# popgenmethods/smcpp

Hardware: AMD Instinct MI355X
Metric: E-step loglik-evals/sec (100 Mbp, M=64, n=20) (higher is better)
Workload: dtype f64 state + f32 scans (mixed)

## Files before the change

smcpp_amd/csrc/chains_ss.hpp:

```cpp
#pragma once

namespace smcpp_dev {

struct SsArgs {
    int M, Mp, nchunks, pass, K, nlds;
    const Chunk *chunks;
    const Chunk *chunks_b;
    int nchunks_b;
    const int *tasks;
    const int2 *rowdesc;
    const double *E;
    const float *pi_f;
    const double *f_dc, *f_g, *f_cg, *f_b, *f_a, *f_d;
    const double *b_dc, *b_g, *b_b, *b_a;
    double c0;
    float *alpha;
    double *beta, *cnorm;
    float *ends_f, *used_f;
    double *ends_b, *used_b;
    int *changed_f, *changed_b;
    int *endchg_f, *endchg_b;
    float eps_f;
    double eps_b;
    int full_f, full_b;
// ... 531 lines not shown
}
#define SS_NBE_ " row_mask:0xf bank_mask:0xf\n"
__device__ __forceinline__ float ss_jump_16(float acc, float X, const float *r) {
    asm volatile("s_nop 1\n"
                 "v_fmac_f32_dpp %0, %1, %2 row_newbcast:0" SS_NBE_ "v_fmac_f32_dpp %0, %1, %3 row_newbcast:1" SS_NBE_
                 "v_fmac_f32_dpp %0, %1, %4 row_newbcast:2" SS_NBE_ "v_fmac_f32_dpp %0, %1, %5 row_newbcast:3" SS_NBE_
                 "v_fmac_f32_dpp %0, %1, %6 row_newbcast:4" SS_NBE_ "v_fmac_f32_dpp %0, %1, %7 row_newbcast:5" SS_NBE_
                 "v_fmac_f32_dpp %0, %1, %8 row_newbcast:6" SS_NBE_ "v_fmac_f32_dpp %0, %1, %9 row_newbcast:7" SS_NBE_
                 "v_fmac_f32_dpp %0, %1, %10 row_newbcast:8" SS_NBE_ "v_fmac_f32_dpp %0, %1, %11 row_newbcast:9" SS_NBE_
                 "v_fmac_f32_dpp %0, %1, %12 row_newbcast:10" SS_NBE_ "v_fmac_f32_dpp %0, %1, %13 row_newbcast:11" SS_NBE_
                 "v_fmac_f32_dpp %0, %1, %14 row_newbcast:12" SS_NBE_ "v_fmac_f32_dpp %0, %1, %15 row_newbcast:13" SS_NBE_
                 "v_fmac_f32_dpp %0, %1, %16 row_newbcast:14" SS_NBE_ "v_fmac_f32_dpp %0, %1, %17 row_newbcast:15" SS_NBE_
                 : "+v"(acc)
                 : "v"(X), "v"(r[0]), "v"(r[1]), "v"(r[2]), "v"(r[3]), "v"(r[4]), "v"(r[5]), "v"(r[6]), "v"(r[7]), "v"(r[8]), "v"(r[9]),
                   "v"(r[10]), "v"(r[11]), "v"(r[12]), "v"(r[13]), "v"(r[14]), "v"(r[15]));
    return acc;
}
#undef SS_NBE_
__device__ __forceinline__ float ss_jump_mv(const SsJumpR &j, float x) {
    const unsigned xi = __builtin_bit_cast(unsigned, x);
    const auto s16 = __builtin_amdgcn_permlane16_swap(xi, xi, false, false);
    const auto sa = __builtin_amdgcn_permlane32_swap(s16[0], s16[0], false, false);
    const auto sb = __builtin_amdgcn_permlane32_swap(s16[1], s16[1], false, false);
    const float a0 = ss_jump_16(0.f, __builtin_bit_cast(float, (unsigned)sa[0]), j.r);
    const float a1 = ss_jump_16(0.f, __builtin_bit_cast(float, (unsigned)sb[0]), j.r + 16);
    const float a2 = ss_jump_16(0.f, __builtin_bit_cast(float, (unsigned)sa[1]), j.r + 32);
    const float a3 = ss_jump_16(0.f, __builtin_bit_cast(float, (unsigned)sb[1]), j.r + 48);
    return (a0 + a1) + (a2 + a3);
}
__device__ __forceinline__ int ss_jump_run(const SsJumpR &j, float &x, int t, int span) {
    const float df = (float)j.d;
    const int nj = (span - t) >> j.sh;
    for (int q = 0; q < nj; ++q) x = __builtin_fmaf(df, x, ss_jump_mv(j, x));
    return t + (nj << (j.sh & 15));
}

__global__ __launch_bounds__(256) void k_ss_jump_tables(SsArgs a, int slot, float *__restrict__ tf, float *__restrict__ tt, double *__restrict__ diag) {
    const int lane = threadIdx.x & 63, i = blockIdx.x * 4 + (threadIdx.x >> 6);
    SsFwdC<1> cst;
    ss_load_fwd<1>(a, lane, cst);
    double e[1], x[1], y[1], S;
    e[0] = a.E[(size_t)slot * 64 + lane];
    x[0] = (lane == i && i < a.M) ? 1.0 : 0.0;
    for (int t = 0; t < a.jump; ++t) {
        ss_fwd_step<1>(cst, x, e, y, S);
        x[0] = y[0];
    }
    const float v = lane == i ? 0.f : (float)x[0];
    tf[lane * 64 + i] = v;
    tt[i * 64 + (63 - lane)] = v;
    if (lane == i) diag[i] = x[0];
}

template <int NPL, bool ALLLDS, bool JMP = false>
__device__ __forceinline__ void ss_fwd_light_rows(const SsArgs &a, const double *sE, long long base, int first, int last, int lane, float (&x)[NPL]);
template <int NPL, bool ALLLDS, bool JMP = false>
__device__ __forceinline__ void ss_bwd_light_rows(const SsArgs &a, const double *sE, long long base, int rhi, int rlo, int lane, float (&b)[NPL]);

template <int NPL, bool RERUN, bool HYB, bool ALLLDS, bool MIX = false, bool H32 = false>
__device__ __forceinline__ void ss_forward_wave(const SsArgs &a, const double *sE, int c, int lane) {
    constexpr int MS = 64 * NPL;
    const int M = a.M, Mp = a.Mp, pass = a.pass;
    const Chunk ch = ss_uniform_chunk(a.chunks[c]);
    float *end_cur = a.ends_f + ((size_t)(pass & 1) * a.nchunks + c) * Mp;
    const float *end_prev = a.ends_f + ((size_t)((pass + 1) & 1) * a.nchunks + c) * Mp;
    int st[NPL];
    bool live[NPL], stor[NPL];
#pragma unroll
    for (int k = 0; k < NPL; ++k) { st[k] = lane * NPL + k; live[k] = st[k] < M; stor[k] = st[k] < Mp; }
    if (RERUN && ch.first && !a.full_f) {
#pragma unroll
        for (int k = 0; k < NPL; ++k) if (stor[k]) end_cur[st[k]] = end_prev[st[k]];
        return;
    }
    double x[NPL];
    {
        const float *src = (ch.first || !RERUN) ? a.pi_f : a.ends_f + ((size_t)((pass + 1) & 1) * a.nchunks + (c - 1)) * Mp;
#pragma unroll
        for (int k = 0; k < NPL; ++k) x[k] = live[k] ? (double)src[st[k]] : 0.0;
    }
    const bool halo = !RERUN && !HYB && a.halo && ch.h0 < ch.r0;
    const int rbeg = halo ? ch.h1 : ch.r0;
    const int jst = ch.r0 - rbeg;
    if (halo && ch.h0 < ch.h1) {
        float xf[NPL];
#pragma unroll
        for (int k = 0; k < NPL; ++k) xf[k] = (float)x[k];
        if (NPL == 1 && !HYB && a.jump) ss_fwd_light_rows<NPL, ALLLDS, NPL == 1 && !HYB>(a, sE, ch.base, ch.h0, ch.h1, lane, xf);
        else ss_fwd_light_rows<NPL, ALLLDS>(a, sE, ch.base, ch.h0, ch.h1, lane, xf);
#pragma unroll
        for (int k = 0; k < NPL; ++k) x[k] = live[k] ? (double)xf[k] : 0.0;
        if (jst == 0) {
            double part = 0.0;
#pragma unroll
            for (int k = 0; k < NPL; ++k) part += x[k];
            const double iv = 1.0 / wave_sum_dpp(part);
#pragma unroll
            for (int k = 0; k < NPL; ++k) {
                const float an = live[k] ? fmaxf((float)(x[k] * iv), ss_floor_at<NPL>(a, ch.base + ch.r0 + 1)) : 0.f;
                x[k] = (double)an;
                if (stor[k]) a.used_f[(size_t)c * Mp + st[k]] = an;
            }
        }
    }
    if (RERUN && !a.full_f) {
        bool diff = false;
#pragma unroll
        for (int k = 0; k < NPL; ++k)
            if (live[k]) {
                const float u = a.used_f[(size_t)c * Mp + st[k]];
                if (!(fabsf((float)x[k] - u) <= a.eps_f * fabsf(u))) diff = true;
            }
        if (!__any(diff)) {
#pragma unroll
            for (int k = 0; k < NPL; ++k) if (stor[k]) end_cur[st[k]] = end_prev[st[k]];
            return;
        }
    }
    if (!halo) {
#pragma unroll
        for (int k = 0; k < NPL; ++k) if (stor[k]) a.used_f[(size_t)c * Mp + st[k]] = (float)x[k];
    }
    if (lane == 0) a.changed_f[pass] = 1;
    if (ch.first) {
#pragma unroll
        for (int k = 0; k < NPL; ++k) if (stor[k]) a.alpha[(size_t)ch.base * Mp + st[k]] = (float)x[k];
        if (lane == 0) a.cnorm[ch.base] = 1.0;
    }
    SsFwdC<NPL> cst;
    ss_load_fwd<NPL>(a, lane, cst);
    SsDescStream rd = ss_desc_stream(a.rowdesc + ch.base + rbeg + 1);
    const int nrows = ch.r1 - rbeg;
    ss_desc_t d1, d2;
    ss_desc_first<1>(rd, d1, d2);
    float *arow = a.alpha + (size_t)(ch.base + rbeg) * Mp;
    double *crow = a.cnorm + ch.base + rbeg;
    float *ap[NPL];
#pragma unroll
    for (int k = 0; k < NPL; ++k) ap[k] = arow + st[k];
    int cacc = 0;
    auto cflush = [&](int jhi) {
        const int jj = (jhi & ~63) + lane;
        if (jj <= jhi && jj > jst && jj > 0) crow[jj] = (double)__builtin_bit_cast(float, cacc);
    };
    double e[NPL];
    ss_emission<NPL, false, ALLLDS>(a, sE, d1.x & 0xFFFF, lane, e);
    constexpr bool hyb = HYB && NPL == 1;
    const double *tab = sE + (size_t)a.nlds * MS;
    SsEigC ec;
    SsHotRows<16> hot;
    int hot_ek = -1;
    if (hyb) {
        ss_load_eig(a, lane, ec);
        if (Mp == 32) { hot_ek = a.hot_ek; ss_eig_rows<16>(ec, tab, Mp, hot_ek, 0, hot.a, hot.b); }
    }
    double *sxw = const_cast<double *>(tab) + (size_t)a.nk_lds * (a.dirsplit ? 2 : 4) * Mp * (Mp + 1) + (threadIdx.x >> 6) * 64;
    bool merged = false;
    const long long t0c = __builtin_readcyclecounter(), t0r = __builtin_amdgcn_s_memrealtime();
    long long npos = 0;
    ss_vm_drain();
    for (int j = 0; j < nrows; ++j) {
        const int jl = j & 63;
        const ss_desc_t d0 = d1;
        d1 = d2; d2 = ss_desc_fetch<1>(rd, d1.x);
        const int span = d0.y;
        const int ekr = (d0.x >> 16) & 0xFF;
        const float flo = NPL >= 2 ? ss_floor_of<NPL>(d0.x) : 1e-10f;
        npos += span;
        if (MIX && jl == 0 && j > 0) cflush(j - 1);
        const int slot_n = d1.x & 0xFFFF;
        double en[NPL];
        ss_emission<NPL, false, ALLLDS>(a, sE, slot_n, lane, en);
        if (hyb && span > a.hyb_th) {
            const double S = wave_sum_dpp(x[0]);
            const double inv = rcp_f64(S);
            double xin = x[0] * inv;
            if (j > 0) {
                const float an = live[0] ? fmaxf((float)xin, flo) : 0.f;
                if (RERUN && !a.full_f && (j & 15) == 0 && j >= 16) {
                    bool bad = false;
                    if (live[0]) {
                        const float old = arow[(size_t)j * Mp + st[0]];
                        if (!(fabsf(an - old) <= a.eps_f * fabsf(old))) bad = true;
                    }
                    if (!__any(bad)) { merged = true; break; }
                }
                if (stor[0]) arow[(size_t)j * Mp + st[0]] = an;
                if (lane == 0) crow[j] = S;
                xin = (double)an;
            }
            const double xo = ss_eig_apply(a, ec, tab, Mp, ekr, 0, sxw, lane, xin, span, hot, hot_ek);
            x[0] = live[0] ? xo : 0.0;
#pragma unroll
            for (int k = 0; k < NPL; ++k) e[k] = en[k];
            continue;
        }
        double y[NPL], S;
        ss_fwd_step<NPL, MIX, MIX && H32>(cst, x, e, y, S);
        double inv;
        if (MIX) {
            const double r0 = (double)__builtin_amdgcn_rcpf((float)S);
            inv = __builtin_fma(__builtin_fma(-S, r0, 1.0), r0, r0);
        } else inv = rcp_f64(S);
        double fb[NPL];
#pragma unroll
        for (int k = 0; k < NPL; ++k) fb[k] = 0.0;
        if (j > 0) {
            float an[NPL];
#pragma unroll
            for (int k = 0; k < NPL; ++k) {
                const double xs = x[k] * inv;
                an[k] = live[k] ? fmaxf((float)xs, flo) : 0.f;
                fb[k] = (double)an[k] - xs;
            }
            if (RERUN && !a.full_f && (j & 15) == 0 && j >= 16) {
                bool bad = false;
#pragma unroll
                for (int k = 0; k < NPL; ++k)
                    if (live[k]) {
                        const float old = MIX ? *ap[k] : arow[(size_t)j * Mp + st[k]];
                        if (!(fabsf(an[k] - old) <= a.eps_f * fabsf(old))) bad = true;
                    }
                if (!__any(bad)) { merged = true; if (MIX) cflush(j - 1); break; }
            }
            if (j > jst) {
                if (MIX) {
#pragma unroll
                    for (int k = 0; k < NPL; ++k) if (stor[k]) *ap[k] = an[k];
                    cacc = lane == jl ? __builtin_bit_cast(int, (float)S) : cacc;
                } else {
#pragma unroll
                    for (int k = 0; k < NPL; ++k) if (stor[k]) arow[(size_t)j * Mp + st[k]] = an[k];
                    if (lane == 0) crow[j] = S;
                }
            } else if (j == jst) {
#pragma unroll
                for (int k = 0; k < NPL; ++k) if (stor[k]) a.used_f[(size_t)c * Mp + st[k]] = an[k];
            }
        }
#pragma unroll
        for (int k = 0; k < NPL; ++k) {
            double ed = e[k] * cst.d[k];
            if (span == 1) { const double edf = (double)(float)ed; y[k] = __builtin_fma(edf - ed, x[k], y[k]); ed = edf; }
            x[k] = __builtin_fma(ed, fb[k], y[k] * inv);
        }
        {
            double S2;
            int t = 1;
            for (; t + 1 < span; t += 2) {
                ss_fwd_step<NPL, MIX, MIX && H32>(cst, x, e, y, S2);
#pragma unroll
                for (int k = 0; k < NPL; ++k) x[k] = y[k];
                ss_fwd_step<NPL, MIX, MIX && H32>(cst, x, e, y, S2);
#pragma unroll
                for (int k = 0; k < NPL; ++k) x[k] = y[k];
            }
            if (t < span) {
                ss_fwd_step<NPL, MIX, MIX && H32>(cst, x, e, y, S2);
#pragma unroll
                for (int k = 0; k < NPL; ++k) x[k] = y[k];
            }
        }
#pragma unroll
        for (int k = 0; k < NPL; ++k) e[k] = en[k];
        if (MIX) {
#pragma unroll
            for (int k = 0; k < NPL; ++k) ap[k] += Mp;
        }
    }
    if (MIX && !merged && nrows > 0) cflush(nrows - 1);
    if (a.dbg && !RERUN && c == 1 && lane == 0) {
        a.dbg[0] = __builtin_readcyclecounter() - t0c; a.dbg[1] = __builtin_amdgcn_s_memrealtime() - t0r;
        a.dbg[2] = npos; a.dbg[3] = nrows;
    }
    if (merged) {
#pragma unroll
        for (int k = 0; k < NPL; ++k) if (stor[k]) end_cur[st[k]] = end_prev[st[k]];
        return;
    }
    {
        double part = 0.0;
#pragma unroll
        for (int k = 0; k < NPL; ++k) part += x[k];
        const double S = wave_sum_dpp(part);
        const double inv = 1.0 / S;
#pragma unroll
        for (int k = 0; k < NPL; ++k) {
            const float an = live[k] ? fmaxf((float)(x[k] * inv), ss_floor_at<NPL>(a, ch.base + ch.r1 + 1)) : 0.f;
            if (stor[k]) { a.alpha[(size_t)(ch.base + ch.r1) * Mp + st[k]] = an; end_cur[st[k]] = an; }
        }
        if (lane == 0) { a.cnorm[ch.base + ch.r1] = S; a.endchg_f[pass] = 1; }
    }
}

template <int NPL, bool RERUN, bool HYB, bool ALLLDS, bool MIX = false, bool H32 = false>
__device__ __forceinline__ void ss_backward_wave(const SsArgs &a, const double *sE, int c, int lane) {
    constexpr int MS = 64 * NPL;
    const int M = a.M, Mp = a.Mp, pass = a.pass;
    const Chunk ch = ss_uniform_chunk(a.chunks_b[c]);
    double *end_cur = a.ends_b + ((size_t)(pass & 1) * a.nchunks_b + c) * Mp;
    const double *end_prev = a.ends_b + ((size_t)((pass + 1) & 1) * a.nchunks_b + c) * Mp;
    int st[NPL];
    bool live[NPL], stor[NPL];
#pragma unroll
    for (int k = 0; k < NPL; ++k) { st[k] = MS - 1 - (lane * NPL + k); live[k] = st[k] < M; stor[k] = st[k] < Mp; }
    if (RERUN && ch.last && !a.full_b) {
#pragma unroll
        for (int k = 0; k < NPL; ++k) if (stor[k]) end_cur[st[k]] = end_prev[st[k]];
        return;
    }
    double b[NPL];
    {
        const bool fresh = ch.last || !RERUN;
        const double *src = a.ends_b + ((size_t)((pass + 1) & 1) * a.nchunks_b + (fresh ? c : c + 1)) * Mp;
#pragma unroll
        for (int k = 0; k < NPL; ++k) b[k] = live[k] ? (fresh ? 1.0 / (double)M : src[st[k]]) : 0.0;
    }
    const bool halo = !RERUN && !HYB && a.halo && ch.h0 > ch.r1;
    const int rend = halo ? ch.h1 : ch.r1;
    const int jst = rend - ch.r1;
    if (halo && ch.h0 > ch.h1) {
        float bf_[NPL];
#pragma unroll
        for (int k = 0; k < NPL; ++k) bf_[k] = (float)b[k];
        if (NPL == 1 && !HYB && a.jump) ss_bwd_light_rows<NPL, ALLLDS, NPL == 1 && !HYB>(a, sE, ch.base, ch.h0, ch.h1, lane, bf_);
        else ss_bwd_light_rows<NPL, ALLLDS>(a, sE, ch.base, ch.h0, ch.h1, lane, bf_);
        float pt = 0.f;
#pragma unroll
        for (int k = 0; k < NPL; ++k) pt += live[k] ? bf_[k] : 0.f;
        const float iv = 1.f / wave_sum_dpp(pt);
#pragma unroll
        for (int k = 0; k < NPL; ++k) b[k] = live[k] ? (double)(bf_[k] * iv) : 0.0;
    }
    if (RERUN && !a.full_b) {
        bool diff = false;
#pragma unroll
        for (int k = 0; k < NPL; ++k)
            if (live[k]) {
                const double u = a.used_b[(size_t)c * Mp + st[k]];
                if (!(fabs(b[k] - u) <= a.eps_b * fabs(u))) diff = true;
            }
        if (!__any(diff)) {
#pragma unroll
            for (int k = 0; k < NPL; ++k) if (stor[k]) end_cur[st[k]] = end_prev[st[k]];
            return;
        }
    }
    if (!halo) {
#pragma unroll
        for (int k = 0; k < NPL; ++k) if (stor[k]) a.used_b[(size_t)c * Mp + st[k]] = b[k];
    }
    if (lane == 0) a.changed_b[pass] = 1;
    SsBwdC<NPL> cst;
    ss_load_bwd<NPL>(a, lane, cst);
    SsDescStream rd = ss_desc_stream(a.rowdesc + ch.base + rend);
    const int nrows = rend - ch.r0;
    ss_desc_t d1, d2;
    ss_desc_first<-1>(rd, d1, d2);
    double *brow = a.beta + (size_t)(ch.base + rend) * Mp;
    double *bp[NPL];
#pragma unroll
    for (int k = 0; k < NPL; ++k) bp[k] = brow + st[k];
    double e[NPL];
    ss_emission<NPL, true, ALLLDS>(a, sE, d1.x & 0xFFFF, lane, e);
    constexpr bool hyb = HYB && NPL == 1;
    const double *tab = sE + (size_t)a.nlds * MS;
    SsEigC ec;
    SsHotRows<16> hot;
    int hot_ek = -1;
    if (hyb) {
        ss_load_eig(a, 63 - lane, ec);
        if (Mp == 32) { hot_ek = a.hot_ek; ss_eig_rows<16>(ec, tab, Mp, hot_ek, 2, hot.a, hot.b); }
    }
    double *sxw = const_cast<double *>(tab) + (size_t)a.nk_lds * (a.dirsplit ? 2 : 4) * Mp * (Mp + 1) + (threadIdx.x >> 6) * 64;
    bool merged = false;
    const long long t0c = __builtin_readcyclecounter(), t0r = __builtin_amdgcn_s_memrealtime();
    long long npos = 0;
    ss_vm_drain();
    for (int j = 0; j < nrows; ++j) {
        const ss_desc_t d0 = d1;
        d1 = d2; d2 = ss_desc_fetch<-1>(rd, d1.x);
        const int span = d0.y;
        const int ekr = (d0.x >> 16) & 0xFF;
        npos += span;
        const int slot_n = d1.x & 0xFFFF;
        double en[NPL];
        ss_emission<NPL, true, ALLLDS>(a, sE, slot_n, lane, en);
        if (RERUN && !a.full_b && (j & 15) == 0 && j >= 16) {
            bool bad = false;
#pragma unroll
            for (int k = 0; k < NPL; ++k)
                if (live[k]) {
                    const double old = MIX ? *bp[k] : brow[-(ptrdiff_t)j * Mp + st[k]];
                    if (!(fabs(b[k] - old) <= a.eps_b * fabs(old))) bad = true;
                }
            if (!__any(bad)) { merged = true; break; }
        }
        if (halo && j == jst) {
            double part = 0.0;
#pragma unroll
            for (int k = 0; k < NPL; ++k) part += live[k] ? b[k] : 0.0;
            const double iv = 1.0 / wave_sum_dpp(part);
#pragma unroll
            for (int k = 0; k < NPL; ++k) {
                b[k] = live[k] ? b[k] * iv : 0.0;
                if (stor[k]) a.used_b[(size_t)c * Mp + st[k]] = b[k];
            }
        }
        if (j >= jst) {
#pragma unroll
            for (int k = 0; k < NPL; ++k) if (stor[k]) { if (MIX) *bp[k] = b[k]; else brow[-(ptrdiff_t)j * Mp + st[k]] = b[k]; }
        }
        if (hyb && span > a.hyb_th) {
            const double bin = live[0] ? b[0] : 0.0;
            double bo = ss_eig_apply(a, ec, tab, Mp, ekr, 2, sxw, 63 - lane, bin, span, hot, hot_ek);
            bo = live[0] ? bo : 0.0;
            b[0] = bo * rcp_f64(wave_sum_dpp(bo));
#pragma unroll
            for (int k = 0; k < NPL; ++k) e[k] = en[k];
            continue;
        }
        double y[NPL];
        float Sw;
        ss_bwd_step<NPL, MIX, MIX && H32>(cst, b, e, y, Sw);
        const double inv = (double)__builtin_amdgcn_rcpf(Sw);
#pragma unroll
        for (int k = 0; k < NPL; ++k) b[k] = y[k] * inv;
        {
            float S2;
            int t = 1;
            for (; t + 1 < span; t += 2) {
                ss_bwd_step<NPL, MIX, MIX && H32>(cst, b, e, y, S2);
#pragma unroll
                for (int k = 0; k < NPL; ++k) b[k] = y[k];
                ss_bwd_step<NPL, MIX, MIX && H32>(cst, b, e, y, S2);
#pragma unroll
                for (int k = 0; k < NPL; ++k) b[k] = y[k];
            }
            if (t < span) {
                ss_bwd_step<NPL, MIX, MIX && H32>(cst, b, e, y, S2);
#pragma unroll
                for (int k = 0; k < NPL; ++k) b[k] = y[k];
            }
        }
#pragma unroll
        for (int k = 0; k < NPL; ++k) e[k] = en[k];
        if (MIX) {
#pragma unroll
            for (int k = 0; k < NPL; ++k) bp[k] -= Mp;
        }
    }
    if (a.dbg && !RERUN && c == 1 && lane == 0) {
        a.dbg[4] = __builtin_readcyclecounter() - t0c; a.dbg[5] = __builtin_amdgcn_s_memrealtime() - t0r;
        a.dbg[6] = npos; a.dbg[7] = nrows;
    }
    if (merged) {
#pragma unroll
        for (int k = 0; k < NPL; ++k) if (stor[k]) end_cur[st[k]] = end_prev[st[k]];
        return;
    }
    {
        double part = 0.0;
#pragma unroll
        for (int k = 0; k < NPL; ++k) part += live[k] ? b[k] : 0.0;
        const double S = wave_sum_dpp(part);
#pragma unroll
        for (int k = 0; k < NPL; ++k) {
            const double bf = live[k] ? b[k] / S : 0.0;
            if (stor[k]) { end_cur[st[k]] = bf; if (ch.first) a.beta[(size_t)ch.base * Mp + st[k]] = bf; }
        }
        if (lane == 0) a.endchg_b[pass] = 1;
    }
}

template <int NPL>
struct SsLightC { float dc[NPL], g[NPL], cg[NPL], b[NPL], a[NPL], cumA[NPL], lv[6], c15, c31, c0; };

template <int NPL, bool BWD>
__device__ __forceinline__ void ss_load_light(const SsArgs &a, int lane, SsLightC<NPL> &c) {
    double cum = 1.0;
#pragma unroll
    for (int k = 0; k < NPL; ++k) {
        const int p = lane * NPL + k;
        c.dc[k] = (float)(BWD ? a.b_dc[p] : a.f_dc[p]);
        c.g[k] = (float)(BWD ? a.b_g[p] : a.f_g[p]);
        c.cg[k] = BWD ? 0.f : (float)a.f_cg[p];
        c.b[k] = (float)(BWD ? a.b_b[p] : a.f_b[p]);
        const double av = BWD ? a.b_a[p] : a.f_a[p];
        c.a[k] = (float)av;
        cum *= av;
        c.cumA[k] = (float)cum;
    }
    double lv[6];
    ss_levels(cum, lane, lv);
#pragma unroll
    for (int q = 0; q < 6; ++q) c.lv[q] = (float)lv[q];
    const int row = lane >> 4;
// ... 68 lines not shown
    const float LIp = dpp0<DPP_WSHR1>(z_);
    if (NPL == 1) {
        out[0] = e[0] * __builtin_fmaf(c.dc[0], x[0], __builtin_fmaf(c.g[0], S, __builtin_fmaf(c.cg[0], p_, LIp)));
        return;
    }
    const float lex = p_ - lp[NPL - 1];
#pragma unroll
    for (int k = 0; k < NPL; ++k) {
        const float incl = lex + lp[k];
        const float Z = (k == 0) ? LIp : __builtin_fmaf(c.cumA[k - 1 < 0 ? 0 : k - 1], LIp, w[k - 1 < 0 ? 0 : k - 1]);
        out[k] = e[k] * __builtin_fmaf(c.dc[k], x[k], __builtin_fmaf(c.g[k], S, __builtin_fmaf(c.cg[k], incl, Z)));
    }
}

template <int NPL, bool H32 = false>
__device__ __forceinline__ void ss_bwd_step_f(const SsLightC<NPL> &c, const float (&bv)[NPL], const float (&e)[NPL],
                                              float (&out)[NPL], float &Sw) {
    float w[NPL], lg[NPL], u[NPL], lf[NPL];
#pragma unroll
    for (int k = 0; k < NPL; ++k) w[k] = e[k] * bv[k];
    lg[0] = c.g[0] * w[0];
    u[0] = w[0];
    lf[0] = w[0];
#pragma unroll
    for (int k = 1; k < NPL; ++k) {
        lg[k] = __builtin_fmaf(c.g[k], w[k], lg[k - 1]);
        u[k] = __builtin_fmaf(c.a[k], u[k - 1], w[k]);
        lf[k] = lf[k - 1] + w[k];
    }
    float p_ = lg[NPL - 1], z_ = u[NPL - 1], f_ = lf[NPL - 1];
    ss_light_scan3<H32>(p_, z_, f_, c.lv, c.c15, c.c31);
    const float Gtot = lane_get(p_, 63);
    Sw = lane_get(f_, 63);
    const float LIp = dpp0<DPP_WSHR1>(z_);
    if (NPL == 1) {
        out[0] = __builtin_fmaf(c.dc[0], w[0], (Gtot - p_) + __builtin_fmaf(c.c0, f_, c.b[0] * LIp));
        return;
    }
    const float lexg = p_ - lg[NPL - 1], lexf = f_ - lf[NPL - 1];
#pragma unroll
    for (int k = 0; k < NPL; ++k) {
        const float inclG = lexg + lg[k], inclW = lexf + lf[k];
        const float V = (k == 0) ? LIp : __builtin_fmaf(c.cumA[k - 1 < 0 ? 0 : k - 1], LIp, u[k - 1 < 0 ? 0 : k - 1]);
        out[k] = __builtin_fmaf(c.dc[k], w[k], (Gtot - inclG) + __builtin_fmaf(c.c0, inclW, c.b[k] * V));
    }
}

template <int NPL, bool BWD, bool ALLLDS>
__device__ __forceinline__ void ss_emission_f(const SsArgs &a, const double *sE, int slot, int lane, float (&e)[NPL]) {
    double ed[NPL];
    ss_emission<NPL, BWD, ALLLDS>(a, sE, slot, lane, ed);
#pragma unroll
    for (int k = 0; k < NPL; ++k) e[k] = (float)ed[k];
}

template <int NPL, bool ALLLDS, bool JMP>
__device__ __forceinline__ void ss_fwd_light_rows(const SsArgs &a, const double *sE, long long base, int first, int last, int lane,
                                                  float (&x)[NPL]) {
    SsLightC<NPL> cst;
    ss_load_light<NPL, false>(a, lane, cst);
    SsDescStream rd = ss_desc_stream(a.rowdesc + base + first + 1);
    const int nrows = last - first;
    ss_desc_t d1, d2;
    ss_desc_first<1>(rd, d1, d2);
    float e[NPL];
    ss_emission_f<NPL, false, ALLLDS>(a, sE, d1.x & 0xFFFF, lane, e);
    SsJumpR jr;
    jr.P = 0; jr.sh = 31;
    if constexpr (JMP) ss_jump_load<false>(a, lane, jr);
    ss_vm_drain();
    for (int j = 0; j < nrows; ++j) {
        const ss_desc_t d0 = d1;
        d1 = d2; d2 = ss_desc_fetch<1>(rd, d1.x);
        const int span = d0.y;
        const bool jrow = JMP && (d0.x & SS_ROW_JUMP);
        const int slot_n = d1.x & 0xFFFF;
        float en[NPL], y[NPL], S;
        ss_emission_f<NPL, false, ALLLDS>(a, sE, slot_n, lane, en);
        ss_fwd_step_f<NPL>(cst, x, e, y, S);
        const float inv = __builtin_amdgcn_rcpf(S);
#pragma unroll
        for (int k = 0; k < NPL; ++k) x[k] = y[k] * inv;
        float S2;
        int t = 1;
        if constexpr (JMP) { if (__builtin_expect(jrow, 0)) t = ss_jump_run(jr, x[0], t, span); }
        for (; t + 1 < span; t += 2) {
            ss_fwd_step_f<NPL>(cst, x, e, y, S2);
#pragma unroll
            for (int k = 0; k < NPL; ++k) x[k] = y[k];
            ss_fwd_step_f<NPL>(cst, x, e, y, S2);
#pragma unroll
            for (int k = 0; k < NPL; ++k) x[k] = y[k];
        }
        if (t < span) {
            ss_fwd_step_f<NPL>(cst, x, e, y, S2);
#pragma unroll
            for (int k = 0; k < NPL; ++k) x[k] = y[k];
        }
#pragma unroll
        for (int k = 0; k < NPL; ++k) e[k] = en[k];
    }
}
template <int NPL, bool ALLLDS, bool JMP>
__device__ __forceinline__ void ss_bwd_light_rows(const SsArgs &a, const double *sE, long long base, int rhi, int rlo, int lane,
                                                  float (&b)[NPL]) {
    SsLightC<NPL> cst;
    ss_load_light<NPL, true>(a, lane, cst);
    SsDescStream rd = ss_desc_stream(a.rowdesc + base + rhi);
    const int nrows = rhi - rlo;
    ss_desc_t d1, d2;
    ss_desc_first<-1>(rd, d1, d2);
    float e[NPL];
    ss_emission_f<NPL, true, ALLLDS>(a, sE, d1.x & 0xFFFF, lane, e);
    SsJumpR jr;
    jr.P = 0; jr.sh = 31;
    if constexpr (JMP) ss_jump_load<true>(a, lane, jr);
    ss_vm_drain();
    for (int j = 0; j < nrows; ++j) {
        const ss_desc_t d0 = d1;
        d1 = d2; d2 = ss_desc_fetch<-1>(rd, d1.x);
        const int span = d0.y;
        const bool jrow = JMP && (d0.x & SS_ROW_JUMP);
        const int slot_n = d1.x & 0xFFFF;
        float en[NPL], y[NPL], Sw;
        ss_emission_f<NPL, true, ALLLDS>(a, sE, slot_n, lane, en);
        ss_bwd_step_f<NPL>(cst, b, e, y, Sw);
        const float inv = __builtin_amdgcn_rcpf(Sw);
#pragma unroll
        for (int k = 0; k < NPL; ++k) b[k] = y[k] * inv;
        float S2;
        int t = 1;
        if constexpr (JMP) { if (__builtin_expect(jrow, 0)) t = ss_jump_run(jr, b[0], t, span); }
        for (; t + 1 < span; t += 2) {
            ss_bwd_step_f<NPL>(cst, b, e, y, S2);
#pragma unroll
            for (int k = 0; k < NPL; ++k) b[k] = y[k];
            ss_bwd_step_f<NPL>(cst, b, e, y, S2);
#pragma unroll
            for (int k = 0; k < NPL; ++k) b[k] = y[k];
        }
        if (t < span) {
            ss_bwd_step_f<NPL>(cst, b, e, y, S2);
#pragma unroll
            for (int k = 0; k < NPL; ++k) b[k] = y[k];
        }
#pragma unroll
        for (int k = 0; k < NPL; ++k) e[k] = en[k];
    }
}

template <int NPL, bool ALLLDS, bool H32 = false, bool JMP = false>
__device__ __forceinline__ void ss_forward_light(const SsArgs &a, const double *sE, int c, int lane) {
    const int M = a.M, Mp = a.Mp, pass = a.pass;
    const Chunk ch = ss_uniform_chunk(a.chunks[c]);
    float *end_cur = a.ends_f + ((size_t)(pass & 1) * a.nchunks + c) * Mp;
    int st[NPL];
    bool live[NPL], stor[NPL];
#pragma unroll
    for (int k = 0; k < NPL; ++k) { st[k] = lane * NPL + k; live[k] = st[k] < M; stor[k] = st[k] < Mp; }
    float x[NPL];
    {
        const float *src = (ch.first || pass == 0) ? a.pi_f : a.ends_f + ((size_t)((pass + 1) & 1) * a.nchunks + (c - 1)) * Mp;
#pragma unroll
        for (int k = 0; k < NPL; ++k) x[k] = live[k] ? src[st[k]] : 0.f;
    }
    if (lane == 0) { a.changed_f[pass] = 1; a.endchg_f[pass] = 1; }
    SsLightC<NPL> cst;
    ss_load_light<NPL, false>(a, lane, cst);
    SsDescStream rd = ss_desc_stream(a.rowdesc + ch.base + ch.r0 + 1);
    const int nrows = ch.r1 - ch.r0;
    ss_desc_t d1, d2;
    ss_desc_first<1>(rd, d1, d2);
    float e[NPL];
    ss_emission_f<NPL, false, ALLLDS>(a, sE, d1.x & 0xFFFF, lane, e);
    SsJumpR jr;
    jr.P = 0; jr.sh = 31;
    if constexpr (JMP) ss_jump_load<false>(a, lane, jr);
    ss_vm_drain();
    for (int j = 0; j < nrows; ++j) {
        const ss_desc_t d0 = d1;
        d1 = d2; d2 = ss_desc_fetch<1>(rd, d1.x);
        const int span = d0.y;
        const bool jrow = JMP && (d0.x & SS_ROW_JUMP);
        const int slot_n = d1.x & 0xFFFF;
        float en[NPL], y[NPL], S;
        ss_emission_f<NPL, false, ALLLDS>(a, sE, slot_n, lane, en);
        ss_fwd_step_f<NPL, H32>(cst, x, e, y, S);
        const float inv = __builtin_amdgcn_rcpf(S);
#pragma unroll
        for (int k = 0; k < NPL; ++k) x[k] = y[k] * inv;
        {
            float S2;
            int t = 1;
            if constexpr (JMP) { if (__builtin_expect(jrow, 0)) t = ss_jump_run(jr, x[0], t, span); }
            for (; t + 1 < span; t += 2) {
                ss_fwd_step_f<NPL, H32>(cst, x, e, y, S2);
#pragma unroll
                for (int k = 0; k < NPL; ++k) x[k] = y[k];
                ss_fwd_step_f<NPL, H32>(cst, x, e, y, S2);
#pragma unroll
                for (int k = 0; k < NPL; ++k) x[k] = y[k];
            }
            if (t < span) {
                ss_fwd_step_f<NPL, H32>(cst, x, e, y, S2);
#pragma unroll
                for (int k = 0; k < NPL; ++k) x[k] = y[k];
            }
        }
#pragma unroll
        for (int k = 0; k < NPL; ++k) e[k] = en[k];
    }
    float part = 0.f;
#pragma unroll
    for (int k = 0; k < NPL; ++k) part += x[k];
    const float inv = 1.f / wave_sum_dpp(part);
#pragma unroll
    for (int k = 0; k < NPL; ++k) if (stor[k]) end_cur[st[k]] = live[k] ? fmaxf(x[k] * inv, ss_floor_at<NPL>(a, ch.base + ch.r1 + 1)) : 0.f;
}

template <int NPL, bool ALLLDS, bool H32 = false, bool JMP = false>
__device__ __forceinline__ void ss_backward_light(const SsArgs &a, const double *sE, int c, int lane) {
    constexpr int MS = 64 * NPL;
    const int M = a.M, Mp = a.Mp, pass = a.pass;
    const Chunk ch = ss_uniform_chunk(a.chunks_b[c]);
    double *end_cur = a.ends_b + ((size_t)(pass & 1) * a.nchunks_b + c) * Mp;
    int st[NPL];
    bool live[NPL], stor[NPL];
#pragma unroll
    for (int k = 0; k < NPL; ++k) { st[k] = MS - 1 - (lane * NPL + k); live[k] = st[k] < M; stor[k] = st[k] < Mp; }
    float b[NPL];
    {
        const bool fresh = ch.last || pass == 0;
        const double *src = a.ends_b + ((size_t)((pass + 1) & 1) * a.nchunks_b + (fresh ? c : c + 1)) * Mp;
#pragma unroll
        for (int k = 0; k < NPL; ++k) b[k] = live[k] ? (fresh ? 1.f / (float)M : (float)src[st[k]]) : 0.f;
    }
    if (lane == 0) { a.changed_b[pass] = 1; a.endchg_b[pass] = 1; }
    SsLightC<NPL> cst;
    ss_load_light<NPL, true>(a, lane, cst);
    SsDescStream rd = ss_desc_stream(a.rowdesc + ch.base + ch.r1);
    const int nrows = ch.r1 - ch.r0;
    ss_desc_t d1, d2;
    ss_desc_first<-1>(rd, d1, d2);
    float e[NPL];
    ss_emission_f<NPL, true, ALLLDS>(a, sE, d1.x & 0xFFFF, lane, e);
    SsJumpR jr;
    jr.P = 0; jr.sh = 31;
    if constexpr (JMP) ss_jump_load<true>(a, lane, jr);
    ss_vm_drain();
    for (int j = 0; j < nrows; ++j) {
        const ss_desc_t d0 = d1;
        d1 = d2; d2 = ss_desc_fetch<-1>(rd, d1.x);
        const int span = d0.y;
        const bool jrow = JMP && (d0.x & SS_ROW_JUMP);
        const int slot_n = d1.x & 0xFFFF;
        float en[NPL], y[NPL], Sw;
        ss_emission_f<NPL, true, ALLLDS>(a, sE, slot_n, lane, en);
        ss_bwd_step_f<NPL, H32>(cst, b, e, y, Sw);
        const float inv = __builtin_amdgcn_rcpf(Sw);
#pragma unroll
        for (int k = 0; k < NPL; ++k) b[k] = y[k] * inv;
        {
            float S2;
            int t = 1;
            if constexpr (JMP) { if (__builtin_expect(jrow, 0)) t = ss_jump_run(jr, b[0], t, span); }
            for (; t + 1 < span; t += 2) {
                ss_bwd_step_f<NPL, H32>(cst, b, e, y, S2);
#pragma unroll
                for (int k = 0; k < NPL; ++k) b[k] = y[k];
                ss_bwd_step_f<NPL, H32>(cst, b, e, y, S2);
#pragma unroll
                for (int k = 0; k < NPL; ++k) b[k] = y[k];
            }
            if (t < span) {
                ss_bwd_step_f<NPL, H32>(cst, b, e, y, S2);
#pragma unroll
                for (int k = 0; k < NPL; ++k) b[k] = y[k];
            }
        }
#pragma unroll
        for (int k = 0; k < NPL; ++k) e[k] = en[k];
    }
    float part = 0.f;
#pragma unroll
    for (int k = 0; k < NPL; ++k) part += live[k] ? b[k] : 0.f;
    const float inv = 1.f / wave_sum_dpp(part);
#pragma unroll
    for (int k = 0; k < NPL; ++k) if (stor[k]) end_cur[st[k]] = live[k] ? (double)(b[k] * inv) : 0.0;
}

template <int NPL, bool HYB, bool ALLLDS, bool H32 = false>
__global__ __launch_bounds__(HYB ? 512 : 256, (NPL == 1 && !HYB) ? 4 : 1) void k_chain_ss(SsArgs a) {
    constexpr int MS = 64 * NPL;
    extern __shared__ __attribute__((aligned(16))) double ss_lds[];
    const int tid = threadIdx.x, lane = tid & 63, w = tid >> 6;
    const bool idle_f = (a.mode_f == 1 && !a.full_f && a.changed_f[a.pass - 1] == 0);
    const bool idle_b = (a.mode_b == 1 && !a.full_b && a.changed_b[a.pass - 1] == 0);
    if (idle_f && idle_b) return;
    const int nthr = HYB ? (int)blockDim.x : 256;
    for (int idx = tid; idx < a.nlds * MS; idx += nthr) ss_lds[idx] = a.E[idx];
    if (HYB && NPL == 1) {
        double *tab = ss_lds + (size_t)a.nlds * MS;
        const int Mp = a.Mp, MM = Mp * Mp;
        if (a.dirsplit) {
            const int nw = nthr >> 6;
            int t0 = -1;
            for (int i = 0; i < nw && t0 < 0; ++i) t0 = a.tasks[nw * blockIdx.x + i];
            const bool wg_bwd = t0 >= 0 && (t0 >> 30);
            for (int idx = tid; idx < a.nk_lds * 2 * MM; idx += nthr) {
                const int mat = idx / MM, rc = idx % MM, r = rc / Mp, cc = rc % Mp;
                const int e = a.key_of_slot[mat >> 1], which = (mat & 1) + (wg_bwd ? 2 : 0);
                const double *src = which == 0 ? a.Pinvrm : which == 1 ? a.Prm : which == 2 ? a.PT : a.PinvT;
                tab[((size_t)mat * Mp + r) * (Mp + 1) + cc] = src[(size_t)e * MM + rc];
            }
        } else
        for (int idx = tid; idx < a.nk_lds * 4 * MM; idx += nthr) {
            const int mat = idx / MM, rc = idx % MM, r = rc / Mp, cc = rc % Mp;
            const int e = a.key_of_slot[mat >> 2], which = mat & 3;
            const double *src = which == 0 ? a.Pinvrm : which == 1 ? a.Prm : which == 2 ? a.PT : a.PinvT;
            tab[((size_t)mat * Mp + r) * (Mp + 1) + cc] = src[(size_t)e * MM + rc];
        }
    }
    __syncthreads();
    const int task = ss_uni(a.tasks[(nthr >> 6) * blockIdx.x + w]);
    if (task < 0) return;
    const bool fwd = !(task >> 30);
    const int c = task & 0x3FFFFFFF;
    if (fwd) {
        if (idle_f) return;
        if (NPL == 1 && !HYB && a.mixed) {
            if (a.mode_f == 0) ss_forward_wave<NPL, false, HYB, ALLLDS, true, H32>(a, ss_lds, c, lane);
            else if (a.mode_f == 1) ss_forward_wave<NPL, true, HYB, ALLLDS, true, H32>(a, ss_lds, c, lane);
            else if (NPL == 1 && !HYB && a.jump) ss_forward_light<NPL, ALLLDS, H32, NPL == 1 && !HYB>(a, ss_lds, c, lane);
            else ss_forward_light<NPL, ALLLDS, H32>(a, ss_lds, c, lane);
        } else
// ... 401 lines not shown
```

Baseline: 1228.

## Restructure SS chain inner loops: unroll-by-4 positions, branch hints, span-1 row batching

Introduces a shared ss_positions helper that unrolls per-position HMM steps by four for NPL==1 (by two otherwise), and a unified ss_light_walk used by all light forward/backward row walkers. For NPL==1 that walker runs consecutive span-1 rows in a tight do-while before entering the position loop, which shortens the per-row control path. Rare branches get __builtin_expect hints, and the early-merge exit becomes a jump to the last row instead of a break, which keeps the loop structure simpler for the compiler. The intent is to cut branch and scalar-control overhead in the dominant scan loops, at the cost of more code and some risk from the reworked merge and jst bookkeeping.

```diff
diff --git a/smcpp_amd/csrc/chains_ss.hpp b/smcpp_amd/csrc/chains_ss.hpp
--- a/smcpp_amd/csrc/chains_ss.hpp
+++ b/smcpp_amd/csrc/chains_ss.hpp
@@ -607,6 +607,31 @@
     if (lane == i) diag[i] = x[0];
 }
 
+template <int NPL, typename F>
+__device__ __forceinline__ void ss_positions(int n, F &&step) {
+    if constexpr (NPL > 1) {
+        int t = 0;
+        for (; t + 1 < n; t += 2) { step(); step(); }
+        if (t < n) step();
+    } else {
+        if (n >= 4) {
+            int q = n >> 2;
+            do { step(); step(); step(); step(); } while (--q > 0);
+        }
+        const int r = n & 3;
+        if (r >= 1) {
+            step();
+            if (r >= 2) {
+                step();
+                if (r == 3) step();
+            }
+        }
+    }
+}
+#define SS_INL_ __attribute__((always_inline))
+#define SS_RARE_(c) (NPL == 1 ? (bool)__builtin_expect((bool)(c), 0) : (bool)(c))
+#define SS_USUAL_(c) (NPL == 1 ? (bool)__builtin_expect((bool)(c), 1) : (bool)(c))
+
 template <int NPL, bool ALLLDS, bool JMP = false>
 __device__ __forceinline__ void ss_fwd_light_rows(const SsArgs &a, const double *sE, long long base, int first, int last, int lane, float (&x)[NPL]);
 template <int NPL, bool ALLLDS, bool JMP = false>
@@ -636,7 +661,7 @@
     }
     const bool halo = !RERUN && !HYB && a.halo && ch.h0 < ch.r0;
     const int rbeg = halo ? ch.h1 : ch.r0;
-    const int jst = ch.r0 - rbeg;
+    int jst = ch.r0 - rbeg;
     if (halo && ch.h0 < ch.h1) {
         float xf[NPL];
 #pragma unroll
@@ -722,7 +747,7 @@
         const int ekr = (d0.x >> 16) & 0xFF;
         const float flo = NPL >= 2 ? ss_floor_of<NPL>(d0.x) : 1e-10f;
         npos += span;
-        if (MIX && jl == 0 && j > 0) cflush(j - 1);
+        if (MIX && __builtin_expect(jl == 0 && j > 0, 0)) { asm volatile(""); cflush(j - 1); }
         const int slot_n = d1.x & 0xFFFF;
         double en[NPL];
         ss_emission<NPL, false, ALLLDS>(a, sE, slot_n, lane, en);
@@ -738,7 +763,7 @@
                         const float old = arow[(size_t)j * Mp + st[0]];
                         if (!(fabsf(an - old) <= a.eps_f * fabsf(old))) bad = true;
                     }
-                    if (!__any(bad)) { merged = true; break; }
+                    if (!__any(bad)) { merged = true; j = nrows - 1; continue; }
                 }
                 if (stor[0]) arow[(size_t)j * Mp + st[0]] = an;
                 if (lane == 0) crow[j] = S;
@@ -760,7 +785,7 @@
         double fb[NPL];
 #pragma unroll
         for (int k = 0; k < NPL; ++k) fb[k] = 0.0;
-        if (j > 0) {
+        if (SS_USUAL_(j > 0)) {
             float an[NPL];
 #pragma unroll
             for (int k = 0; k < NPL; ++k) {
@@ -768,7 +793,7 @@
                 an[k] = live[k] ? fmaxf((float)xs, flo) : 0.f;
                 fb[k] = (double)an[k] - xs;
             }
-            if (RERUN && !a.full_f && (j & 15) == 0 && j >= 16) {
+            if (RERUN && SS_RARE_(!a.full_f && (j & 15) == 0 && j >= 16)) {
                 bool bad = false;
 #pragma unroll
                 for (int k = 0; k < NPL; ++k)
@@ -776,9 +801,13 @@
                         const float old = MIX ? *ap[k] : arow[(size_t)j * Mp + st[k]];
                         if (!(fabsf(an[k] - old) <= a.eps_f * fabsf(old))) bad = true;
                     }
-                if (!__any(bad)) { merged = true; if (MIX) cflush(j - 1); break; }
-            }
-            if (j > jst) {
+                if (!__any(bad)) {
+                    merged = true;
+                    if (MIX) cflush(j - 1);
+                    if constexpr (NPL == 1) { j = nrows - 1; jst = nrows; } else break;
+                }
+            }
+            if (SS_USUAL_(j > jst)) {
                 if (MIX) {
 #pragma unroll
                     for (int k = 0; k < NPL; ++k) if (stor[k]) *ap[k] = an[k];
@@ -788,7 +817,11 @@
                     for (int k = 0; k < NPL; ++k) if (stor[k]) arow[(size_t)j * Mp + st[k]] = an[k];
                     if (lane == 0) crow[j] = S;
                 }
-            } else if (j == jst) {
+            } else if (NPL > 1 && j == jst) {
+#pragma unroll
+                for (int k = 0; k < NPL; ++k) if (stor[k]) a.used_f[(size_t)c * Mp + st[k]] = an[k];
+            }
+            if (NPL == 1 && halo && __builtin_expect(j == jst, 0)) {
 #pragma unroll
                 for (int k = 0; k < NPL; ++k) if (stor[k]) a.used_f[(size_t)c * Mp + st[k]] = an[k];
             }
@@ -799,23 +832,13 @@
             if (span == 1) { const double edf = (double)(float)ed; y[k] = __builtin_fma(edf - ed, x[k], y[k]); ed = edf; }
             x[k] = __builtin_fma(ed, fb[k], y[k] * inv);
         }
-        {
-            double S2;
-            int t = 1;
-            for (; t + 1 < span; t += 2) {
+        if (NPL > 1 || __builtin_expect(span > 1, 0))
+            ss_positions<NPL>(span - 1, [&]() SS_INL_ {
+                double S2;
                 ss_fwd_step<NPL, MIX, MIX && H32>(cst, x, e, y, S2);
 #pragma unroll
                 for (int k = 0; k < NPL; ++k) x[k] = y[k];
-                ss_fwd_step<NPL, MIX, MIX && H32>(cst, x, e, y, S2);
-#pragma unroll
-                for (int k = 0; k < NPL; ++k) x[k] = y[k];
-            }
-            if (t < span) {
-                ss_fwd_step<NPL, MIX, MIX && H32>(cst, x, e, y, S2);
-#pragma unroll
-                for (int k = 0; k < NPL; ++k) x[k] = y[k];
-            }
-        }
+            });
 #pragma unroll
         for (int k = 0; k < NPL; ++k) e[k] = en[k];
         if (MIX) {
@@ -873,7 +896,7 @@
     }
     const bool halo = !RERUN && !HYB && a.halo && ch.h0 > ch.r1;
     const int rend = halo ? ch.h1 : ch.r1;
-    const int jst = rend - ch.r1;
+    int jst = rend - ch.r1;
     if (halo && ch.h0 > ch.h1) {
         float bf_[NPL];
 #pragma unroll
@@ -941,7 +964,7 @@
         const int slot_n = d1.x & 0xFFFF;
         double en[NPL];
         ss_emission<NPL, true, ALLLDS>(a, sE, slot_n, lane, en);
-        if (RERUN && !a.full_b && (j & 15) == 0 && j >= 16) {
+        if (RERUN && SS_RARE_(!a.full_b && (j & 15) == 0 && j >= 16)) {
             bool bad = false;
 #pragma unroll
             for (int k = 0; k < NPL; ++k)
@@ -949,9 +972,12 @@
                     const double old = MIX ? *bp[k] : brow[-(ptrdiff_t)j * Mp + st[k]];
                     if (!(fabs(b[k] - old) <= a.eps_b * fabs(old))) bad = true;
                 }
-            if (!__any(bad)) { merged = true; break; }
-        }
-        if (halo && j == jst) {
+            if (!__any(bad)) {
+                merged = true;
+                if constexpr (NPL == 1) { j = nrows - 1; jst = nrows; } else break;
+            }
+        }
+        if (halo && SS_RARE_(j == jst)) {
             double part = 0.0;
 #pragma unroll
             for (int k = 0; k < NPL; ++k) part += live[k] ? b[k] : 0.0;
@@ -962,7 +988,7 @@
                 if (stor[k]) a.used_b[(size_t)c * Mp + st[k]] = b[k];
             }
         }
-        if (j >= jst) {
+        if (SS_USUAL_(j >= jst)) {
 #pragma unroll
             for (int k = 0; k < NPL; ++k) if (stor[k]) { if (MIX) *bp[k] = b[k]; else brow[-(ptrdiff_t)j * Mp + st[k]] = b[k]; }
         }
@@ -981,23 +1007,13 @@
         const double inv = (double)__builtin_amdgcn_rcpf(Sw);
 #pragma unroll
         for (int k = 0; k < NPL; ++k) b[k] = y[k] * inv;
-        {
-            float S2;
-            int t = 1;
-            for (; t + 1 < span; t += 2) {
+        if (NPL > 1 || __builtin_expect(span > 1, 0))
+            ss_positions<NPL>(span - 1, [&]() SS_INL_ {
+                float S2;
                 ss_bwd_step<NPL, MIX, MIX && H32>(cst, b, e, y, S2);
 #pragma unroll
                 for (int k = 0; k < NPL; ++k) b[k] = y[k];
-                ss_bwd_step<NPL, MIX, MIX && H32>(cst, b, e, y, S2);
-#pragma unroll
-                for (int k = 0; k < NPL; ++k) b[k] = y[k];
-            }
-            if (t < span) {
-                ss_bwd_step<NPL, MIX, MIX && H32>(cst, b, e, y, S2);
-#pragma unroll
-                for (int k = 0; k < NPL; ++k) b[k] = y[k];
-            }
-        }
+            });
 #pragma unroll
         for (int k = 0; k < NPL; ++k) e[k] = en[k];
         if (MIX) {
@@ -1172,6 +1188,66 @@
     ss_emission<NPL, BWD, ALLLDS>(a, sE, slot, lane, ed);
 #pragma unroll
     for (int k = 0; k < NPL; ++k) e[k] = (float)ed[k];
+}
+
+template <int NPL, bool BWD, bool ALLLDS, bool H32, bool JMP>
+__device__ __forceinline__ void ss_light_walk(const SsArgs &a, const double *sE, SsDescStream rd, ss_desc_t d1, ss_desc_t d2, int nrows,
+                                              int lane, const SsLightC<NPL> &cst, const SsJumpR &jr, float (&e)[NPL], float (&v)[NPL]) {
+    auto step = [&](const float (&em)[NPL], float (&y)[NPL], float &S) SS_INL_ {
+        if constexpr (BWD) ss_bwd_step_f<NPL, H32>(cst, v, em, y, S);
+        else ss_fwd_step_f<NPL, H32>(cst, v, em, y, S);
+    };
+    if constexpr (NPL > 1) {
+        for (int j = 0; j < nrows; ++j) {
+            const ss_desc_t d0 = d1;
+            d1 = d2; d2 = ss_desc_fetch<BWD ? -1 : 1>(rd, d1.x);
+            const int span = d0.y;
+            const int slot_n = d1.x & 0xFFFF;
+            float en[NPL], y[NPL], S;
+            ss_emission_f<NPL, BWD, ALLLDS>(a, sE, slot_n, lane, en);
+            step(e, y, S);
+            const float inv = __builtin_amdgcn_rcpf(S);
+#pragma unroll
+            for (int k = 0; k < NPL; ++k) v[k] = y[k] * inv;
+            ss_positions<NPL>(span - 1, [&]() SS_INL_ {
+                float S2;
+                step(e, y, S2);
+#pragma unroll
+                for (int k = 0; k < NPL; ++k) v[k] = y[k];
+            });
+#pragma unroll
+            for (int k = 0; k < NPL; ++k) e[k] = en[k];
+        }
+        return;
+    }
+    int j = 0;
+    while (j < nrows) {
+        int span;
+        bool jrow;
+        float ep[NPL], y[NPL];
+        do {
+            const ss_desc_t d0 = d1;
+            d1 = d2; d2 = ss_desc_fetch<BWD ? -1 : 1>(rd, d1.x);
+            span = d0.y;
+            jrow = JMP && (d0.x & SS_ROW_JUMP);
+            const int slot_n = d1.x & 0xFFFF;
+            float en[NPL], S;
+            ss_emission_f<NPL, BWD, ALLLDS>(a, sE, slot_n, lane, en);
+            step(e, y, S);
+            const float inv = __builtin_amdgcn_rcpf(S);
+#pragma unroll
+            for (int k = 0; k < NPL; ++k) { v[k] = y[k] * inv; ep[k] = e[k]; e[k] = en[k]; }
+            ++j;
+        } while ((span == 1) & (j < nrows));
+        int t = 1;
+        if constexpr (JMP) { if (__builtin_expect(jrow, 0)) t = ss_jump_run(jr, v[0], t, span); }
+        ss_positions<NPL>(span - t, [&]() SS_INL_ {
+            float S2;
+            step(ep, y, S2);
+#pragma unroll
+            for (int k = 0; k < NPL; ++k) v[k] = y[k];
+        });
+    }
 }
 
 template <int NPL, bool ALLLDS, bool JMP>
@@ -1189,37 +1265,7 @@
     jr.P = 0; jr.sh = 31;
     if constexpr (JMP) ss_jump_load<false>(a, lane, jr);
     ss_vm_drain();
-    for (int j = 0; j < nrows; ++j) {
-        const ss_desc_t d0 = d1;
-        d1 = d2; d2 = ss_desc_fetch<1>(rd, d1.x);
-        const int span = d0.y;
-        const bool jrow = JMP && (d0.x & SS_ROW_JUMP);
-        const int slot_n = d1.x & 0xFFFF;
-        float en[NPL], y[NPL], S;
-        ss_emission_f<NPL, false, ALLLDS>(a, sE, slot_n, lane, en);
-        ss_fwd_step_f<NPL>(cst, x, e, y, S);
-        const float inv = __builtin_amdgcn_rcpf(S);
-#pragma unroll
-        for (int k = 0; k < NPL; ++k) x[k] = y[k] * inv;
-        float S2;
-        int t = 1;
-        if constexpr (JMP) { if (__builtin_expect(jrow, 0)) t = ss_jump_run(jr, x[0], t, span); }
-        for (; t + 1 < span; t += 2) {
-            ss_fwd_step_f<NPL>(cst, x, e, y, S2);
-#pragma unroll
-            for (int k = 0; k < NPL; ++k) x[k] = y[k];
-            ss_fwd_step_f<NPL>(cst, x, e, y, S2);
-#pragma unroll
-            for (int k = 0; k < NPL; ++k) x[k] = y[k];
-        }
-        if (t < span) {
-            ss_fwd_step_f<NPL>(cst, x, e, y, S2);
-#pragma unroll
-            for (int k = 0; k < NPL; ++k) x[k] = y[k];
-        }
-#pragma unroll
-        for (int k = 0; k < NPL; ++k) e[k] = en[k];
-    }
+    ss_light_walk<NPL, false, ALLLDS, false, JMP>(a, sE, rd, d1, d2, nrows, lane, cst, jr, e, x);
 }
 template <int NPL, bool ALLLDS, bool JMP>
 __device__ __forceinline__ void ss_bwd_light_rows(const SsArgs &a, const double *sE, long long base, int rhi, int rlo, int lane,
@@ -1236,37 +1282,7 @@
     jr.P = 0; jr.sh = 31;
     if constexpr (JMP) ss_jump_load<true>(a, lane, jr);
     ss_vm_drain();
-    for (int j = 0; j < nrows; ++j) {
-        const ss_desc_t d0 = d1;
-        d1 = d2; d2 = ss_desc_fetch<-1>(rd, d1.x);
-        const int span = d0.y;
-        const bool jrow = JMP && (d0.x & SS_ROW_JUMP);
-        const int slot_n = d1.x & 0xFFFF;
-        float en[NPL], y[NPL], Sw;
-        ss_emission_f<NPL, true, ALLLDS>(a, sE, slot_n, lane, en);
-        ss_bwd_step_f<NPL>(cst, b, e, y, Sw);
-        const float inv = __builtin_amdgcn_rcpf(Sw);
-#pragma unroll
-        for (int k = 0; k < NPL; ++k) b[k] = y[k] * inv;
-        float S2;
-        int t = 1;
-        if constexpr (JMP) { if (__builtin_expect(jrow, 0)) t = ss_jump_run(jr, b[0], t, span); }
-        for (; t + 1 < span; t += 2) {
-            ss_bwd_step_f<NPL>(cst, b, e, y, S2);
-#pragma unroll
-            for (int k = 0; k < NPL; ++k) b[k] = y[k];
-            ss_bwd_step_f<NPL>(cst, b, e, y, S2);
-#pragma unroll
-            for (int k = 0; k < NPL; ++k) b[k] = y[k];
-        }
-        if (t < span) {
-            ss_bwd_step_f<NPL>(cst, b, e, y, S2);
-#pragma unroll
-            for (int k = 0; k < NPL; ++k) b[k] = y[k];
-        }
-#pragma unroll
-        for (int k = 0; k < NPL; ++k) e[k] = en[k];
-    }
+    ss_light_walk<NPL, true, ALLLDS, false, JMP>(a, sE, rd, d1, d2, nrows, lane, cst, jr, e, b);
 }
 
 template <int NPL, bool ALLLDS, bool H32 = false, bool JMP = false>
@@ -1297,39 +1313,7 @@
     jr.P = 0; jr.sh = 31;
     if constexpr (JMP) ss_jump_load<false>(a, lane, jr);
     ss_vm_drain();
-    for (int j = 0; j < nrows; ++j) {
-        const ss_desc_t d0 = d1;
-        d1 = d2; d2 = ss_desc_fetch<1>(rd, d1.x);
-        const int span = d0.y;
-        const bool jrow = JMP && (d0.x & SS_ROW_JUMP);
-        const int slot_n = d1.x & 0xFFFF;
-        float en[NPL], y[NPL], S;
-        ss_emission_f<NPL, false, ALLLDS>(a, sE, slot_n, lane, en);
-        ss_fwd_step_f<NPL, H32>(cst, x, e, y, S);
-        const float inv = __builtin_amdgcn_rcpf(S);
-#pragma unroll
-        for (int k = 0; k < NPL; ++k) x[k] = y[k] * inv;
-        {
-            float S2;
-            int t = 1;
-            if constexpr (JMP) { if (__builtin_expect(jrow, 0)) t = ss_jump_run(jr, x[0], t, span); }
-            for (; t + 1 < span; t += 2) {
-                ss_fwd_step_f<NPL, H32>(cst, x, e, y, S2);
-#pragma unroll
-                for (int k = 0; k < NPL; ++k) x[k] = y[k];
-                ss_fwd_step_f<NPL, H32>(cst, x, e, y, S2);
-#pragma unroll
-                for (int k = 0; k < NPL; ++k) x[k] = y[k];
-            }
-            if (t < span) {
-                ss_fwd_step_f<NPL, H32>(cst, x, e, y, S2);
-#pragma unroll
-                for (int k = 0; k < NPL; ++k) x[k] = y[k];
-            }
-        }
-#pragma unroll
-        for (int k = 0; k < NPL; ++k) e[k] = en[k];
-    }
+    ss_light_walk<NPL, false, ALLLDS, H32, JMP>(a, sE, rd, d1, d2, nrows, lane, cst, jr, e, x);
     float part = 0.f;
 #pragma unroll
     for (int k = 0; k < NPL; ++k) part += x[k];
@@ -1368,39 +1352,7 @@
     jr.P = 0; jr.sh = 31;
     if constexpr (JMP) ss_jump_load<true>(a, lane, jr);
     ss_vm_drain();
-    for (int j = 0; j < nrows; ++j) {
-        const ss_desc_t d0 = d1;
-        d1 = d2; d2 = ss_desc_fetch<-1>(rd, d1.x);
-        const int span = d0.y;
-        const bool jrow = JMP && (d0.x & SS_ROW_JUMP);
-        const int slot_n = d1.x & 0xFFFF;
-        float en[NPL], y[NPL], Sw;
-        ss_emission_f<NPL, true, ALLLDS>(a, sE, slot_n, lane, en);
-        ss_bwd_step_f<NPL, H32>(cst, b, e, y, Sw);
-        const float inv = __builtin_amdgcn_rcpf(Sw);
-#pragma unroll
-        for (int k = 0; k < NPL; ++k) b[k] = y[k] * inv;
-        {
-            float S2;
-            int t = 1;
-            if constexpr (JMP) { if (__builtin_expect(jrow, 0)) t = ss_jump_run(jr, b[0], t, span); }
-            for (; t + 1 < span; t += 2) {
-                ss_bwd_step_f<NPL, H32>(cst, b, e, y, S2);
-#pragma unroll
-                for (int k = 0; k < NPL; ++k) b[k] = y[k];
-                ss_bwd_step_f<NPL, H32>(cst, b, e, y, S2);
-#pragma unroll
-                for (int k = 0; k < NPL; ++k) b[k] = y[k];
-            }
-            if (t < span) {
-                ss_bwd_step_f<NPL, H32>(cst, b, e, y, S2);
-#pragma unroll
-                for (int k = 0; k < NPL; ++k) b[k] = y[k];
-            }
-        }
-#pragma unroll
-        for (int k = 0; k < NPL; ++k) e[k] = en[k];
-    }
+    ss_light_walk<NPL, true, ALLLDS, H32, JMP>(a, sE, rd, d1, d2, nrows, lane, cst, jr, e, b);
     float part = 0.f;
 #pragma unroll
     for (int k = 0; k < NPL; ++k) part += live[k] ? b[k] : 0.f;
```

Result: faster. 1289, median of 6 (+5.0%).
